# AberHu/TF-NAS

Measured on AMD Instinct MI355X. Metric: supernet search images/sec (w-step + alpha-step), higher is better.
Workload: dtype fp32

## Files before the change

### tf-nas_amd/csrc/capi.hip

```cpp
#include <string.h>
#include "tfnas_dev.h"
#include "kernels.h"
#include "cell_impl.h"

#include <stdlib.h>
#include <mutex>
#include <vector>

struct SideCtx {
    int device;
    hipStream_t main, side;
    hipEvent_t fork[4], join;
};
static std::mutex g_side_mu;
static std::vector<SideCtx*> g_side;

static SideCtx* side_for(hipStream_t s) {
    int dev = 0;
    if (hipGetDevice(&dev) != hipSuccess) return nullptr;
    std::lock_guard<std::mutex> lk(g_side_mu);
    for (SideCtx* c : g_side)
        if (c->main == s && c->device == dev) return c;
    SideCtx* c = new SideCtx();
    c->device = dev;
// ... 246 lines not shown
    if (bn) TRY(bn_fwd_fix(d0, bn, 1, stats2, s));
    TRY(launch_se_pool(d, b.D, stats2, pooled, s));
    TRY(launch_se_fc_fwd(d, pooled, hpre, gate, b.part, TFNAS_PART_FLOATS, s));
    TRY(launch_project_fwd(d, b.D, gate, stats2, b.Pr, stats3, b.part, s));
    if (sync) TRY(stats_sync(d, stats3, 2 * (size_t)d.G * d.oc, s));
    if (bn) TRY(bn_fwd_fix(d0, bn, 2, stats3, s));
    if (b.drop_scale && d.has_res) {
        TfnasCellDesc dn = dc;
        dn.has_res = 0;
        TRY(launch_mix_fwd(dn, b.Pr, stats3, b.wmix, b.x, b.out, s));
        return launch_rowscale(b.out, b.out, b.x, b.drop_scale, d.N, (uint64_t)d.Ho * d.Wo * d.oc, s);
    }
    TRY(launch_mix_fwd(d, b.Pr, stats3, b.wmix, b.x, b.out, s));
    return 0;
}

static hipStream_t fork_to(const CellSide* so, int k, hipStream_t main) {
    if (!so || !so->side[k] || so->side[k] == main) return main;
    if (hipEventRecord(so->fork[k], main) != hipSuccess || hipStreamWaitEvent(so->side[k], so->fork[k], 0) != hipSuccess)
        return main;
    return so->side[k];
}

static int bn_bwd_fix(const TfnasCellDesc& d, const TfnasBnAffine* bn, int site, double* red, hipStream_t s) {
    int nch;
    uint64_t cnt;
    bn_site(d, site, nch, cnt);
    TRY(launch_bn_bwd_fix(red, nch, cnt, bn->weight[site], bn->bias[site], bn->g_weight[site], bn->g_bias[site], s,
                          wgrad_accum(d)));
    if (bn->eval) return (int)hipMemsetAsync(red, 0, sizeof(double) * 2 * (size_t)nch, s);
    return 0;
}

static int expand_dx(const TfnasCellDesc& d, const float* dEh, const float* x, const float* cb1, float* part, const float* dout,
                     const float* wmix, float* dx, float* dxp, hipStream_t s, const float* add_src = nullptr,
                     const float* add_scale = nullptr, int nsl = -1) {
    const size_t room = TFNAS_PART_FLOATS - expand_gram_floats(d);
    float* gram = part + room;
    TRY(launch_expand_gram(d, cb1, part, room, gram, s));
    return launch_expand_dgrad(d, dEh, x, cb1, gram, dout, wmix, dx, dxp, s, add_src, add_scale, nsl);
}


int cell_bwd_impl(const TfnasCellDesc& d0, const TfnasCellWs& ws, const CellBwdBufs& b0, hipStream_t s, const CellSide* so,
                  int fwd_route) {
    const TfnasBnAffine* bn = b0.bn;
    TfnasCellDesc dc = d0;
    if (bn) dc.eps = -1.f;
    const TfnasCellDesc& d = dc;
    CellBwdBufs b = b0;
    const int taken = route_taken(d0, bn != nullptr);
    if ((fwd_route & TFNAS_ROUTE_TAKEN_VALID) && taken != fwd_route) return TFNAS_EINVAL;
    const float* dout_res = b0.dout;
    if (b0.drop_scale && d.has_res) {
        if (!b0.dout_s) return TFNAS_ENULL;
        TRY(launch_rowscale(b0.dout_s, b0.dout, nullptr, b0.drop_scale, d.N, (uint64_t)d.Ho * d.Wo * d.oc, s));
        b.dout = b0.dout_s;
    }
    const double* stats1 = b.stats + ws.off_stats1;
    const double* stats2 = b.stats + ws.off_stats2;
    const double* stats3 = b.stats + ws.off_stats3;
    const float* pooled = b.fsmall + ws.off_pooled;
    const float* gate = b.fsmall + ws.off_gate;
    const float* hpre = b.fsmall + ws.off_hpre;
    float* dgate = b.bsmall + ws.off_dgate;
    float* dpooled = b.bsmall + ws.off_dpooled;
    float* dhpre = b.bsmall + ws.off_dhpre;
    float* cb1 = b.bsmall + ws.off_cb1;
    double* red3 = b.red + ws.off_red3;
    double* red2 = b.red + ws.off_red2;
    double* red1 = b.red + ws.off_red1;
    float* part = b.part;
    float* part_w = b.part_w;
    float* part_w1 = b.part_w1 ? b.part_w1 : b.part_w;
    float* part_w2 = b.part_w2 ? b.part_w2 : b.part_w;

    if (d.need_wgrad) {
        for (int g = 0; g < d.G; ++g) {
            const TfnasGroup& gr = d.g[g];
            if (!gr.g_expand || !gr.g_dw || !gr.g_proj) return TFNAS_ENULL;
            if (gr.se > 0 && (!gr.g_se_r || !gr.gb_se_r || !gr.g_se_e || !gr.gb_se_e)) return TFNAS_ENULL;
        }
    }
    TRY(launch_mix_bwd_stats(d, b.dout, b.Pr, stats3, b.x, red3, part, s));
    TRY(stats_sync(d, red3, 2 * (size_t)d.G * d.oc, s));
    if (b.dwmix) TRY(launch_mix_dw(d, red3, b.red + ws.off_resdot, b.dwmix, s));
    if (bn) TRY(bn_bwd_fix(d0, bn, 2, red3, s));
    if (!b.dx && !d.need_wgrad) return 0;
    if (d.need_wgrad)
        TRY(launch_project_wgrad(d, b.dout, b.Pr, b.D, gate, stats2, stats3, red3, b.wmix, part_w, fork_to(so, 0, s)));
    const bool fused2 = bn2_fused_fits(d);
    const bool fold = fused2 && !(d.route & TFNAS_ROUTE_FOLD_OFF) && project_fold_ok(d, (size_t)ws.dEh) && (d.G == 1 || d.Ho * d.Wo <= 784);
    if (fold) {
        TRY(launch_project_dgrad(d, b.dout, b.Pr, stats3, red3, b.wmix, b.dZ, s, b.D, stats2, b.dEh));
        TRY(launch_bn2_gather(d, b.dEh, dgate, part, s));
    } else {
        TRY(launch_project_dgrad(d, b.dout, b.Pr, stats3, red3, b.wmix, b.dZ, s));
        if (fused2) TRY(launch_bn2_pool(d, b.dZ, b.D, stats2, dgate, part, s));
        else TRY(launch_se_bwd_reduce(d, b.dZ, b.D, stats2, dgate, s));
    }
    TRY(launch_se_fc_bwd(d, dgate, gate, hpre, dhpre, dpooled, b.dEh, (size_t)ws.dEh, s));
    if (fused2) TRY(launch_bn2_finish(d, part, gate, dpooled, red2, s));
    else TRY(launch_bn2_bwd(d, b.dZ, b.D, stats2, gate, dpooled, red2, part, s));
    TRY(stats_sync(d, red2, 2 * (size_t)d.M, s));
    if (bn) TRY(bn_bwd_fix(d0, bn, 1, red2, s));
    if (taken & TFNAS_ROUTE_TAKEN_FX) {
        int nsl = 0;
        TRY(launch_fx_bwd(d, b.x, b.E, stats1, stats2, red2, b.dZ, b.D, gate, dpooled, b.dEh, (size_t)ws.dEh, red1, cb1, part, &nsl, s));
        if (b.dx) TRY(expand_dx(d, nullptr, b.x, cb1, part, dout_res, b.wmix, b.dx, b.dEh, s, b.add_src, b.add_scale, nsl));
        return 0;
    }
    const DwPlan dw_bwd = dw_plan_bwd_data(d, b.E == nullptr, b.x != nullptr);
    const bool dw_fused = dw_bwd.fuse_wgrad;
    if (d.need_wgrad) {
        if (d.SE > 0 || !dw_fused) {
            hipStream_t sw = fork_to(so, 1, s);
            if (d.SE > 0) TRY(launch_se_wgrad(d, dgate, gate, dhpre, hpre, pooled, sw));
            if (!dw_fused) TRY(launch_dw_wgrad(d, b.dZ, gate, dpooled, b.D, stats2, red2, b.E, stats1, part_w1, sw));
        }
    }
    if (bn || stats_sync_on(d)) {
        TRY(launch_dw_bwd_data(dw_bwd, d, b.dZ, gate, dpooled, b.D, stats2, red2, b.E, b.x, stats1, b.dEh, red1, part, s));
        TRY(stats_sync(d, red1, 2 * (size_t)d.M, s));
        if (bn) TRY(bn_bwd_fix(d0, bn, 0, red1, s));
        TRY(launch_bn1_consts(d, stats1, red1, cb1, s));
    } else {
        TRY(launch_dw_bwd_data(dw_bwd, d, b.dZ, gate, dpooled, b.D, stats2, red2, b.E, b.x, stats1, b.dEh, red1, part, s, cb1));
    }
    if (d.need_wgrad) TRY(launch_expand_wgrad(d, b.dEh, b.E, cb1, b.x, part_w2, fork_to(so, 2, s)));
    if (b.dx && d.mode != TFNAS_MODE_STEM)
        TRY(expand_dx(d, b.dEh, b.x, cb1, part, dout_res, b.wmix, b.dx, b.dxp, s, b.add_src, b.add_scale));
    return 0;
}

extern "C" int tfnas_mixedop_fwd(const TfnasCellDesc* dp, const float* x, const float* wmix, float* E, float* D,
                                 float* Pr, float* fsmall, double* stats, float* part, float* out, void* stream) {
    if (!dp || !x || !D || !Pr || !fsmall || !stats || !part || !out) return TFNAS_ENULL;
    const TfnasCellDesc& d = *dp;
    if (d.mode == TFNAS_MODE_HEAD) return TFNAS_EINVAL;
    if (!E && !efree_supported(d)) return TFNAS_ENULL;
    TRY(check_modes(dp));
    TfnasCellWs ws;
    TRY(tfnas_cell_ws(dp, &ws));
    CellFwdBufs b = {x, wmix, E, D, Pr, fsmall, stats, part, out};
    return cell_fwd_impl(d, ws, b, S(stream));
}

static int cell_bwd_entry(const TfnasCellDesc& d, CellBwdBufs b, hipStream_t s, void* const* wgrad_stream, bool lazy) {
    TfnasCellWs ws;
    TRY(tfnas_cell_ws(&d, &ws));
    SideCtx* sc = (d.need_wgrad && route_side(d)) ? side_for(s) : nullptr;
    SideJoinGuard guard;
    guard.c = sc;
    guard.main = s;
    CellSide so = {};
    if (sc) {
        for (int i = 0; i < 3; ++i) {
            hipStream_t own = (wgrad_stream && wgrad_stream[i]) ? S(wgrad_stream[i]) : nullptr;
            so.side[i] = own ? own : sc->side;
            guard.extra[i] = own;
            so.fork[i] = sc->fork[i];
            if (own) {
                b.part_w1 = b.part + 2 * TFNAS_PART_ALLOC;
                b.part_w2 = b.part + 3 * TFNAS_PART_ALLOC;
            }
        }
    }
// ... 195 lines not shown
```

### tf-nas_amd/csrc/kernels.h

```cpp
#pragma once
#include <stdlib.h>
#include <hip/hip_runtime.h>
#include "tfnas_hip.h"

struct StatsSync {
    tfnas_stats_sync_fn fn;
    void* user;
    int world;
};
extern StatsSync g_stats_sync;
static inline StatsSync sync_of(const TfnasCellDesc& d) {
    if (d.sync_fn) return StatsSync{d.sync_fn, d.sync_user, d.sync_world > 0 ? d.sync_world : 1};
    return g_stats_sync;
}
static inline bool stats_sync_on(const TfnasCellDesc& d) { return sync_of(d).fn != nullptr; }
static inline int stats_sync(const TfnasCellDesc& d, double* table, size_t ndoubles, hipStream_t s) {
    const StatsSync y = sync_of(d);
    return y.fn ? y.fn(y.user, table, (uint64_t)ndoubles, (void*)s) : 0;
}
static inline uint64_t stats_world(const TfnasCellDesc& d) {
    const StatsSync y = sync_of(d);
    return (y.fn && y.world > 1) ? (uint64_t)y.world : 1;
}

// ... 35 lines not shown
                         const double* red3, const float* wmix, float* dZ, hipStream_t s, const float* D = nullptr,
                         const double* stats2 = nullptr, float* rec = nullptr);
constexpr int FOLD_SLOTS = 4, FOLD_Q = 5;
static inline bool project_fold_ok(const TfnasCellDesc& d, size_t scratch_floats) {
    const int HW = d.Ho * d.Wo;
    const size_t nrt = ((size_t)d.N * HW + 127) / 128;
    return HW >= 43 && nrt * FOLD_SLOTS * FOLD_Q * (size_t)d.M <= scratch_floats;
}
int launch_project_wgrad(const TfnasCellDesc& d, const float* dout, const float* Pr, const float* D,
                         const float* gate, const double* stats2, const double* stats3, const double* red3,
                         const float* wmix, float* part, hipStream_t s);
size_t expand_gram_floats(const TfnasCellDesc& d);
int launch_expand_gram(const TfnasCellDesc& d, const float* cb1, float* scratch, size_t scratch_floats, float* gram,
                       hipStream_t s);
int launch_expand_dgrad(const TfnasCellDesc& d, const float* dEh, const float* x, const float* cb1, const float* gram,
                        const float* dout, const float* wmix, float* dx, float* dxp, hipStream_t s,
                        const float* add_src = nullptr, const float* add_scale = nullptr, int nsl = -1);
int launch_expand_wgrad(const TfnasCellDesc& d, const float* dEh, const float* E, const float* cb1,
                        const float* x, float* part, hipStream_t s);

struct DwDirect {
    int chunks;
    int ncg;
    int nseg;
    int per;
    int steps;
    int nwg;
};
struct DwSlide {
    int TH, TW;
    int CC, CCP, cq_shift;
    int RB, L1;
    int chunks, gx;
};
struct DwGeom {
    int T0, T1;
    int CC;
    int cq_shift;
    int tilesH, tilesW, ntiles;
    int L0, L1;
};
enum DwFamily { DW_DIRECT, DW_RING, DW_TILE };
struct DwPlan {
    DwFamily fam;
    int rows;
    int chunks[2];
    DwDirect direct[2];
    DwSlide ring[2];
    DwGeom tile[2];
    int jw;
    bool pipe;
    int kq;
    bool fuse_wgrad;
};
int launch_dw_fwd(const TfnasCellDesc& d, const float* E, const float* x, const double* stats1, float* D,
                  double* stats2, float* part, hipStream_t s);
bool efree_supported(const TfnasCellDesc& d);
static inline bool efree_ic_ok(int ic) { return ic == 16 || ic == 24 || ic == 40; }
int launch_expand_stats_gram(const TfnasCellDesc& d, const float* x, double* stats1, float* part, hipStream_t s);
int launch_x_colsum(const float* x, int P, int ic, int rps, int nb, float* part, hipStream_t s);
bool fx_supported(const TfnasCellDesc& d);
int launch_fx_stats(const TfnasCellDesc& d, const float* x, double* stats1, float* part, hipStream_t s);
int launch_fx_fwd(const TfnasCellDesc& d, const float* x, const double* stats1, float* E, float* D, double* stats2,
                  float* part, hipStream_t s);
int launch_fx_bwd(const TfnasCellDesc& d, const float* x, const float* Eh, const double* stats1, const double* stats2,
                  const double* red2, const float* dZ, const float* D, const float* gate, const float* dpooled, float* scratch,
                  size_t scratch_floats, double* red1, float* cb1, float* part, int* nsl, hipStream_t s);
DwPlan dw_plan_bwd_data(const TfnasCellDesc& d, bool efree, bool has_x);
int launch_dw_bwd_data(const DwPlan& p, const TfnasCellDesc& d, const float* dZ, const float* gate, const float* dpooled,
                       const float* D, const double* stats2, const double* red2, const float* E, const float* x,
                       const double* stats1, float* dEh, double* red1, float* part, hipStream_t s, float* cb1 = nullptr);
int launch_reduce_bn1(const TfnasCellDesc& d, const float* part, int nb, const double* stats1, double* red1, float* cb1,
                      hipStream_t s);
int launch_dw_wgrad(const TfnasCellDesc& d, const float* dZ, const float* gate, const float* dpooled, const float* D,
                    const double* stats2,
                    const double* red2, const float* E, const double* stats1, float* part, hipStream_t s);

int launch_se_pool(const TfnasCellDesc& d, const float* D, const double* stats2, float* pooled, hipStream_t s);
int launch_se_fc_fwd(const TfnasCellDesc& d, const float* pooled, float* hpre, float* gate, float* scratch,
                     size_t scratch_floats, hipStream_t s);
int launch_mix_fwd(const TfnasCellDesc& d, const float* Pr, const double* stats3, const float* wmix,
                   const float* x, float* out, hipStream_t s);
int launch_mix_bwd_stats(const TfnasCellDesc& d, const float* dout, const float* Pr, const double* stats3,
                         const float* x, double* red3, float* part, hipStream_t s);
int launch_mix_dw(const TfnasCellDesc& d, const double* red3, const double* resdot, float* dwmix, hipStream_t s);
int launch_se_bwd_reduce(const TfnasCellDesc& d, const float* dZ, const float* D, const double* stats2,
                         float* dgate, hipStream_t s);
int launch_se_fc_bwd(const TfnasCellDesc& d, const float* dgate, const float* gate, const float* hpre, float* dhpre,
                     float* dpooled, float* scratch, size_t scratch_floats, hipStream_t s);
int launch_se_wgrad(const TfnasCellDesc& d, const float* dgate, const float* gate, const float* dhpre,
                    const float* hpre, const float* pooled, hipStream_t s);
bool bn2_fused_fits(const TfnasCellDesc& d);
int launch_bn2_pool(const TfnasCellDesc& d, const float* dZ, const float* D, const double* stats2, float* dgate,
                    float* pp, hipStream_t s);
int launch_bn2_gather(const TfnasCellDesc& d, const float* rec, float* dgate, float* pp, hipStream_t s);
int launch_bn2_finish(const TfnasCellDesc& d, const float* pp, const float* gate, const float* dpooled, double* red2,
                      hipStream_t s);
int launch_bn2_bwd(const TfnasCellDesc& d, const float* dZ, const float* D, const double* stats2, const float* gate,
                   const float* dpooled, double* red2, float* part, hipStream_t s);
int launch_head_pool(const TfnasCellDesc& d, const float* E, const double* stats1, float* pooled, hipStream_t s);
int launch_head_bwd(const TfnasCellDesc& d, const float* E, const double* stats1, const float* dpooled, float* dEh,
                    double* red1, float* part, hipStream_t s);
int launch_reduce_rows(const float* part, int nb, int ncols, size_t stride, double* out_d, float* out_f,
                       hipStream_t s, int accum = 0);
#define TFNAS_PART_ALLOC ((size_t)4 << 20)
#define TFNAS_TAIL_SLOTS ((size_t)1024)
#define TFNAS_PART_FLOATS (TFNAS_PART_ALLOC - TFNAS_TAIL_SLOTS)
int launch_bn1_consts(const TfnasCellDesc& d, const double* stats1, const double* red1, float* cb1,
                      hipStream_t s);

int launch_arch_fwd(int ncell, const float* const* la, const float* e, const float* lat, float T, float* w,
                    float* cell_lat, hipStream_t s);
int launch_arch_bwd(int ncell, const float* w, const float* lat, const float* dw, const float* dcl, float T,
                    float* const* dla, hipStream_t s);
int launch_arch_project(int n, float* const* p, const int32_t* len, hipStream_t s);
int launch_arch_sample(int ncell, const float* const* la, const uint8_t* mask, const float* e, float T, int mode,
                       int32_t* pos, hipStream_t s);
int launch_sink_fwd(int K, const float* betas, const float* const* res, const float* cell_lat, uint64_t count,
                    float* out, float* out_lat, float* bw, hipStream_t s);
int launch_scale_copy(float* dst, const float* src, const float* scale, uint64_t count, hipStream_t s);
int launch_sink_bwd(int K, const float* bw, const float* const* res, const float* cell_lat, const float* dout,
                    const float* dlat, uint64_t count, float* const* dres, float* dbetas, float* dcell_lat,
                    double* dots, hipStream_t s);

int launch_pack_ranges(const float* src, float* dst, int nranges, const uint64_t* off, const uint64_t* doff,
                       const uint64_t* len, hipStream_t s);
int launch_sgd_clip_step(float* w, float* g, float* m, int nranges, const uint64_t* off, const uint64_t* goff,
                         const uint64_t* len, float max_norm,
                         float lr, float momentum, float wd, float grad_scale, double* scratch, uint64_t scratch_doubles,
                         float* norm_out, hipStream_t s);
int launch_arch_adam_project(int n, float* const* p, const float* const* g, const int32_t* len, float* m, float* v,
                             float max_norm, float lr, float b1, float b2, float eps, float wd, int step, float grad_scale,
                             float* norm_out, hipStream_t s);

int launch_bn_fwd_fix(double* stats, int nch, uint64_t cnt, float eps, const float* gamma, const float* beta, float* rmean,
                      float* rvar, float momentum, int eval, hipStream_t s, uint64_t world = 1);
int launch_bn_bwd_fix(double* red, int nch, uint64_t cnt, const float* gamma, const float* beta, float* dgamma, float* dbeta,
                      hipStream_t s, int accum = 0);
int launch_rowscale(float* out, const float* y, const float* res, const float* scale, int N, uint64_t per_image,
                    hipStream_t s);
```

### tf-nas_amd/csrc/pointwise_kernels.hip

```cpp
#include "tfnas_dev.h"
#include "kernels.h"
#include "prof.h"

__device__ __forceinline__ f32x4 reduce_rows(f32x4 v, f32x4* buf, int pr, int col, int RP, int TQ, bool active) {
    __syncthreads();
    if (active) buf[pr * TQ + col] = v;
    __syncthreads();
    int s = 1;
    while (s * 2 < RP) s *= 2;
    for (; s > 0; s >>= 1) {
        if (active && pr < s && pr + s < RP) buf[pr * TQ + col] += buf[(pr + s) * TQ + col];
        __syncthreads();
    }
    return (active && pr == 0) ? buf[col] : zero4();
}

__device__ __forceinline__ bool chunk_locate(const TfnasCellDesc& d, int cy, int CH, bool se_only, int& g, int& c0) {
    for (g = 0; g < d.G; ++g) {
        if (se_only && d.g[g].se == 0) continue;
        const int t = (d.g[g].mcp + CH - 1) / CH;
        if (cy < t) {
            c0 = cy * CH;
            return true;
        }
// ... 9 lines not shown
}
#ifndef TFNAS_POOL_ROWS
#define TFNAS_POOL_ROWS 4
#endif
constexpr int PU = TFNAS_POOL_ROWS;
template <int ACT, int MODE>
__global__ __launch_bounds__(256) void k_se_pool(TfnasCellDesc d, const float* __restrict__ D,
                                                 const double* __restrict__ stats2, const float* __restrict__ dZ,
                                                 float* __restrict__ outp) {
    __shared__ f32x4 buf[256];
    int g, c0;
    if (!chunk_locate(d, blockIdx.y, 64, true, g, c0)) return;
    const int mc = d.g[g].mc, mcp = d.g[g].mcp, off = d.g[g].off;
    const int HW = d.Ho * d.Wo, M = d.M, n = blockIdx.x;
    const int nq = (min(64, mcp - c0) + 3) >> 2, cqs = nq <= 4 ? 2 : (nq <= 8 ? 3 : 4), CQN = 1 << cqs, RLN = 256 >> cqs;
    const int tid = threadIdx.x, cq = tid & (CQN - 1), rl = tid >> cqs;
    const int ch = c0 + 4 * cq;
    const bool active = ch < mcp;
    float2 c2[4];
#pragma unroll
    for (int j = 0; j < 4; ++j)
        c2[j] = (active && ch + j < mc) ? bn_consts(stats2 + 2 * (size_t)(off + ch + j), 1.0 / ((double)d.N * HW), d.eps)
                                        : make_float2(0.f, 0.f);
    f32x4 acc = zero4();
    if (active) {
        for (int hw = rl; hw < HW; hw += PU * RLN) {
            f32x4 v[PU], z[PU];
#pragma unroll
            for (int u = 0; u < PU; ++u) {
                const int h = hw + RLN * u;
                const size_t a = ((size_t)n * HW + (h < HW ? h : 0)) * M + off + ch;
                v[u] = ld4_nt(D + a);
                z[u] = (MODE == 1) ? ld4_nt(dZ + a) : zero4();
            }
#pragma unroll
            for (int u = 0; u < PU; ++u) {
                if (hw + RLN * u < HW) {
#pragma unroll
                    for (int j = 0; j < 4; ++j) v[u][j] = act_f<ACT>((v[u][j] - c2[j].x) * c2[j].y);
                    acc += (MODE == 1) ? v[u] * z[u] : v[u];
                }
            }
        }
    }
    acc = reduce_rows(acc, buf, rl, cq, RLN, CQN, active);
    if (active && rl == 0) {
        if (MODE == 0) acc *= splat4(1.f / (float)HW);
        st4(outp + (size_t)n * M + off + ch, acc);
    }
}

__global__ __launch_bounds__(256) void k_mix_fwd(TfnasCellDesc d, const float* __restrict__ Pr,
                                                 const double* __restrict__ stats3, const float* __restrict__ wmix,
                                                 const float* __restrict__ x, float* __restrict__ out) {
    extern __shared__ __attribute__((aligned(16))) float lds[];
    float2* tab = reinterpret_cast<float2*>(lds);
    const int oc = d.oc, G = d.G, OQ = oc >> 2;
    const int Po = d.N * d.Ho * d.Wo;
    float sumw = 0.f;
    for (int g = 0; g < G; ++g) sumw += wmix ? wmix[g] : 1.f;
    for (int i = threadIdx.x; i < G * oc; i += 256) {
        const float2 c = bn_consts(stats3 + 2 * (size_t)i, 1.0 / (double)Po, d.eps);
        tab[i] = make_float2(c.x, c.y * (wmix ? wmix[i / oc] : 1.f));
    }
    __syncthreads();
    const size_t total = (size_t)Po * OQ;
    for (size_t idx = (size_t)blockIdx.x * 256 + threadIdx.x; idx < total; idx += (size_t)gridDim.x * 256) {
        const size_t p = idx / OQ;
        const int o = (int)(idx % OQ) * 4;
        f32x4 v = zero4();
        for (int g = 0; g < G; ++g) {
            const f32x4 pr = ld4(Pr + ((size_t)g * Po + p) * oc + o);
#pragma unroll
            for (int j = 0; j < 4; ++j) {
                const float2 t = tab[g * oc + o + j];
                v[j] += (pr[j] - t.x) * t.y;
            }
        }
        if (d.has_res) v += splat4(sumw) * ld4(x + p * d.ic + o);
        st4(out + p * oc + o, v);
    }
}

__global__ __launch_bounds__(256) void k_mix_bwd_stats(TfnasCellDesc d, const float* __restrict__ dout,
                                                       const float* __restrict__ Pr,
                                                       const double* __restrict__ stats3,
                                                       const float* __restrict__ x, float* __restrict__ part,
                                                       int rows_per_block) {
    extern __shared__ __attribute__((aligned(16))) float lds[];
    const int oc = d.oc, TQ = oc >> 2, RP = 256 / TQ;
    const int Po = d.N * d.Ho * d.Wo;
    const int G = d.G, Gall = d.G;
    float2* tab = reinterpret_cast<float2*>(lds);
    f32x4* buf = reinterpret_cast<f32x4*>(lds + 2 * Gall * oc);
    for (int i = threadIdx.x; i < G * oc; i += 256) tab[i] = bn_consts(stats3 + 2 * (size_t)i, 1.0 / (double)Po, d.eps);
    __syncthreads();
    const int tid = threadIdx.x, oq = tid % TQ, pr = tid / TQ, o = 4 * oq;
    const bool active = pr < RP;
    const int p0 = blockIdx.x * rows_per_block, p1 = min(Po, p0 + rows_per_block);
    f32x4 s1 = zero4(), sx = zero4(), s2[TFNAS_MAX_GROUPS];
#pragma unroll
    for (int g = 0; g < TFNAS_MAX_GROUPS; ++g) s2[g] = zero4();
    if (active) {
        for (int p = p0 + pr; p < p1; p += RP) {
            const f32x4 dv = ld4(dout + (size_t)p * oc + o);
            s1 += dv;
            if (d.has_res) sx += dv * ld4(x + (size_t)p * d.ic + o);
#pragma unroll
            for (int g = 0; g < TFNAS_MAX_GROUPS; ++g) {
                if (g < G) {
                    const f32x4 pv = ld4(Pr + ((size_t)g * Po + p) * oc + o);
#pragma unroll
                    for (int j = 0; j < 4; ++j) {
                        const float2 t = tab[g * oc + o + j];
                        s2[g][j] += dv[j] * ((pv[j] - t.x) * t.y);
                    }
                }
            }
        }
    }
    float* prow = part + (size_t)blockIdx.x * (2 * Gall * oc + oc);
    s1 = reduce_rows(s1, buf, pr, oq, RP, TQ, active);
    sx = reduce_rows(sx, buf, pr, oq, RP, TQ, active);
    if (active && pr == 0) st4(prow + 2 * Gall * oc + o, sx);
#pragma unroll
    for (int g = 0; g < TFNAS_MAX_GROUPS; ++g) {
        if (g < G) {
            const f32x4 r = reduce_rows(s2[g], buf, pr, oq, RP, TQ, active);
            if (active && pr == 0) {
#pragma unroll
                for (int j = 0; j < 4; ++j) {
                    prow[2 * ((size_t)g * oc + o + j) + 0] = s1[j];
                    prow[2 * ((size_t)g * oc + o + j) + 1] = r[j];
                }
            }
        }
    }
}

__global__ __launch_bounds__(64) void k_mix_dw(TfnasCellDesc d, const double* __restrict__ red3, const double* __restrict__ resdot,
                                               float* __restrict__ dwmix) {
    const int g = blockIdx.x, lane = threadIdx.x;
    double s = 0.0;
    for (int o = lane; o < d.oc; o += 64) {
        s += red3[2 * ((size_t)g * d.oc + o) + 1];
        if (d.has_res) s += resdot[o];
    }
#pragma unroll
    for (int m = 32; m > 0; m >>= 1) s += __shfl_xor(s, m, 64);
    if (lane == 0) dwmix[g] = (float)s;
}

template <int ACT>
__global__ __launch_bounds__(256) void k_bn2_pool(TfnasCellDesc d, const float* __restrict__ dZ, const float* __restrict__ D,
                                                  const double* __restrict__ stats2, float* __restrict__ dgate,
                                                  float* __restrict__ pp, int CH) {
    __shared__ f32x4 buf[256];
    int g, c0;
    if (!chunk_locate(d, blockIdx.y, CH, false, g, c0)) return;
    const int mc = d.g[g].mc, mcp = d.g[g].mcp, off = d.g[g].off;
    const bool has_se = d.g[g].se > 0;
    const int HW = d.Ho * d.Wo, M = d.M, n = blockIdx.x;
    const int nq = (min(CH, mcp - c0) + 3) >> 2, cqs = nq <= 4 ? 2 : (nq <= 8 ? 3 : 4), CQN = 1 << cqs, RLN = 256 >> cqs;
    const int tid = threadIdx.x, cq = tid & (CQN - 1), rl = tid >> cqs;
    const int ch = c0 + 4 * cq;
    const bool active = ch < mcp;
    float2 c2[4];
#pragma unroll
    for (int j = 0; j < 4; ++j)
        c2[j] = (active && ch + j < mc) ? bn_consts(stats2 + 2 * (size_t)(off + ch + j), 1.0 / ((double)d.N * HW), d.eps)
                                        : make_float2(0.f, 0.f);
    f32x4 g0 = zero4(), a1 = zero4(), b1 = zero4(), a2 = zero4(), b2 = zero4();
    if (active) {
        for (int hw = rl; hw < HW; hw += PU * RLN) {
            f32x4 v[PU], z[PU];
#pragma unroll
            for (int u = 0; u < PU; ++u) {
                const int h = hw + RLN * u;
                const size_t a = ((size_t)n * HW + (h < HW ? h : 0)) * M + off + ch;
                v[u] = ld4_nt(D + a);
                z[u] = ld4_nt(dZ + a);
            }
#pragma unroll
            for (int u = 0; u < PU; ++u) {
                if (hw + RLN * u < HW) {
#pragma unroll
                    for (int j = 0; j < 4; ++j) {
                        const float dh = (v[u][j] - c2[j].x) * c2[j].y;
                        const float ad = act_d<ACT>(dh), zd = z[u][j] * ad;
                        a1[j] += zd;
                        b1[j] += zd * dh;
                        if (has_se) {
                            g0[j] += z[u][j] * act_f<ACT>(dh);
                            a2[j] += ad;
                            b2[j] += ad * dh;
                        }
                    }
                }
            }
        }
    }
    const size_t NM = (size_t)d.N * M, o = (size_t)n * M + off + ch;
    a1 = reduce_rows(a1, buf, rl, cq, RLN, CQN, active);
    if (active && rl == 0) st4(pp + o, a1);
    b1 = reduce_rows(b1, buf, rl, cq, RLN, CQN, active);
    if (active && rl == 0) st4(pp + NM + o, b1);
    if (has_se) {
        a2 = reduce_rows(a2, buf, rl, cq, RLN, CQN, active);
        if (active && rl == 0) st4(pp + 2 * NM + o, a2);
        b2 = reduce_rows(b2, buf, rl, cq, RLN, CQN, active);
        if (active && rl == 0) st4(pp + 3 * NM + o, b2);
        g0 = reduce_rows(g0, buf, rl, cq, RLN, CQN, active);
        if (active && rl == 0) st4(dgate + o, g0);
    }
}

__global__ __launch_bounds__(256) void k_bn2_gather(TfnasCellDesc d, const float* __restrict__ rec, float* __restrict__ dgate,
                                                    float* __restrict__ pp) {
// ... 389 lines not shown
    __syncthreads();
    if (tid < CL / 2) {
        const int ch = blockIdx.x * (CL / 2) + tid;
        if (ch < d.M) {
            const double inv = 1.0 / ((double)d.N * d.H * d.W);
            const float2 m = bn_consts(stats1 + 2 * (size_t)ch, inv, d.eps);
            f32x4 t;
            t.x = m.x;
            t.y = m.y;
            t.z = (float)(tot[2 * tid] * inv);
            t.w = (float)(tot[2 * tid + 1] * inv);
            bool is_pad = true;
            for (int g = 0; g < d.G; ++g)
                if (ch >= d.g[g].off && ch < d.g[g].off + d.g[g].mc) is_pad = false;
            if (is_pad) t = zero4();
            reinterpret_cast<f32x4*>(cb1)[ch] = t;
        }
    }
}

int launch_reduce_bn1(const TfnasCellDesc& d, const float* part, int nb, const double* stats1, double* red1, float* cb1,
                      hipStream_t s) {
    ProfScope _prof(TK_REDUCE_ROWS, s);
    hipLaunchKernelGGL(k_reduce_bn1, dim3(cdiv(2 * d.M, 16)), dim3(256), 0, s, d, part, nb, stats1, red1, cb1);
    return (int)hipGetLastError();
}

int launch_reduce_rows(const float* part, int nb, int ncols, size_t stride, double* out_d, float* out_f,
                       hipStream_t s, int accum) {
    ProfScope _prof(TK_REDUCE_ROWS, s);
    const bool al4 = (ncols & 3) == 0 && (stride & 3) == 0 && ((uintptr_t)part & 15) == 0;
    const size_t in_stride = 0, out_stride = 0;
    if (al4 && nb <= 128 && ncols >= 1024)
        hipLaunchKernelGGL(k_reduce_rows_wide, dim3(cdiv(ncols, 128), 1), dim3(256), 0, s, part, nb, ncols, stride, out_d,
                           out_f, in_stride, out_stride, accum);
    else if (al4 && nb > 64)
        hipLaunchKernelGGL(k_reduce_rows_q<4>, dim3(cdiv(ncols, 16), 1), dim3(256), 0, s, part, nb, ncols, stride, out_d, out_f,
                           in_stride, out_stride, accum);
    else if (ncols <= 2048 && nb > 256)
        hipLaunchKernelGGL(k_reduce_rows<4>, dim3(cdiv(ncols, 4), 1), dim3(256), 0, s, part, nb, ncols, stride, out_d, out_f,
                           in_stride, out_stride, accum);
    else
        hipLaunchKernelGGL(k_reduce_rows<8>, dim3(cdiv(ncols, 8), 1), dim3(256), 0, s, part, nb, ncols, stride, out_d, out_f,
                           in_stride, out_stride, accum);
    return (int)hipGetLastError();
}

int launch_se_pool(const TfnasCellDesc& d, const float* D, const double* stats2, float* pooled, hipStream_t s) {
    ProfScope _prof(TK_SE_POOL, s);
    const int chunks = chunk_count(d, 64, true);
    if (!chunks) return 0;
    dim3 grid(d.N, chunks);
    ACT_DISPATCH(d.act, {
        hipLaunchKernelGGL((k_se_pool<ACT, 0>), grid, dim3(256), 0, s, d, D, stats2, (const float*)nullptr, pooled);
    })
    return (int)hipGetLastError();
}

int launch_se_bwd_reduce(const TfnasCellDesc& d, const float* dZ, const float* D, const double* stats2,
                         float* dgate, hipStream_t s) {
    ProfScope _prof(TK_SE_BWD_REDUCE, s);
    const int chunks = chunk_count(d, 64, true);
    if (!chunks) return 0;
    dim3 grid(d.N, chunks);
    ACT_DISPATCH(d.act, {
        hipLaunchKernelGGL((k_se_pool<ACT, 1>), grid, dim3(256), 0, s, d, D, stats2, dZ, dgate);
    })
    return (int)hipGetLastError();
}

int launch_mix_fwd(const TfnasCellDesc& d, const float* Pr, const double* stats3, const float* wmix,
                   const float* x, float* out, hipStream_t s) {
    ProfScope _prof(TK_MIX_FWD, s);
    const size_t total = (size_t)d.N * d.Ho * d.Wo * (d.oc / 4);
    size_t blocks = cdiv64(total, 256 * 4);
    if (blocks > 4096) blocks = 4096;
    if (blocks < 1) blocks = 1;
    const size_t shm = (size_t)2 * d.G * d.oc * sizeof(float);
    hipLaunchKernelGGL(k_mix_fwd, dim3((unsigned)blocks), dim3(256), shm, s, d, Pr, stats3, wmix, x, out);
    return (int)hipGetLastError();
}

int launch_mix_bwd_stats(const TfnasCellDesc& d, const float* dout, const float* Pr, const double* stats3,
                         const float* x, double* red3, float* part, hipStream_t s) {
    ProfScope _prof(TK_MIX_BWD_STATS, s);
    const int Po = d.N * d.Ho * d.Wo;
    const int ncols = 2 * d.G * d.oc + d.oc;
    size_t nblk = 1024;
    if (nblk > TFNAS_PART_FLOATS / (size_t)ncols) nblk = TFNAS_PART_FLOATS / (size_t)ncols;
    int rpb = cdiv(Po, (int)nblk);
    const int RP = 256 / (d.oc / 4);
    if (rpb < 8 * RP) rpb = 8 * RP;
    const size_t shm = (size_t)(2 * d.G * d.oc + 4 * 256) * sizeof(float);
    const int gx = cdiv(Po, rpb);
    hipLaunchKernelGGL(k_mix_bwd_stats, dim3(gx), dim3(256), shm, s, d, dout, Pr, stats3, x, part, rpb);
    _prof.stop();
    return launch_reduce_rows(part, gx, ncols, (size_t)ncols, red3, nullptr, s);
}

int launch_mix_dw(const TfnasCellDesc& d, const double* red3, const double* resdot, float* dwmix, hipStream_t s) {
    ProfScope _prof(TK_SMALL, s);
    hipLaunchKernelGGL(k_mix_dw, dim3(d.G), dim3(64), 0, s, d, red3, resdot, dwmix);
    return (int)hipGetLastError();
}

int launch_bn2_bwd(const TfnasCellDesc& d, const float* dZ, const float* D, const double* stats2, const float* gate,
                   const float* dpooled, double* red2, float* part, hipStream_t s) {
    ProfScope _prof(TK_BN2_BWD, s);
    const int Po = d.N * d.Ho * d.Wo;
    const int chunks = chunk_count(d, 64, false);
    int want = cdiv(4096, chunks);
    if (want > 1024) want = 1024;
    const size_t cap = TFNAS_PART_FLOATS / (2 * (size_t)d.M);
    if ((size_t)want > cap) want = (int)cap;
    int rpb = cdiv(Po, want < 1 ? 1 : want);
    if (rpb < 64) rpb = 64;
    dim3 grid(cdiv(Po, rpb), chunks);
    ACT_DISPATCH(d.act, {
        hipLaunchKernelGGL((k_bn2_bwd<ACT>), grid, dim3(256), 0, s, d, dZ, D, stats2, gate, dpooled, part, rpb);
    })
    _prof.stop();
    return launch_reduce_rows(part, grid.x, 2 * d.M, 2 * (size_t)d.M, red2, nullptr, s);
}

bool bn2_fused_fits(const TfnasCellDesc& d) { return 4 * (size_t)d.N * d.M <= TFNAS_PART_FLOATS; }

int launch_bn2_pool(const TfnasCellDesc& d, const float* dZ, const float* D, const double* stats2, float* dgate,
                    float* pp, hipStream_t s) {
    ProfScope _prof(TK_SE_BWD_REDUCE, s);
    const int CH = (d.N * chunk_count(d, 64, false) < 1024 && d.Ho * d.Wo >= 196) ? 32 : 64;
    dim3 grid(d.N, chunk_count(d, CH, false));
    ACT_DISPATCH(d.act, { hipLaunchKernelGGL((k_bn2_pool<ACT>), grid, dim3(256), 0, s, d, dZ, D, stats2, dgate, pp, CH); })
    return (int)hipGetLastError();
}

int launch_bn2_gather(const TfnasCellDesc& d, const float* rec, float* dgate, float* pp, hipStream_t s) {
    ProfScope _prof(TK_SE_BWD_REDUCE, s);
    hipLaunchKernelGGL(k_bn2_gather, dim3(d.N, chunk_count(d, 64, false)), dim3(256), 0, s, d, rec, dgate, pp);
    return (int)hipGetLastError();
}

int launch_bn2_finish(const TfnasCellDesc& d, const float* pp, const float* gate, const float* dpooled, double* red2,
                      hipStream_t s) {
    ProfScope _prof(TK_BN2_BWD, s);
    hipLaunchKernelGGL(k_bn2_finish, dim3(chunk_count(d, 64, false)), dim3(256), 0, s, d, pp, gate, dpooled, red2);
    return (int)hipGetLastError();
}

int launch_head_pool(const TfnasCellDesc& d, const float* E, const double* stats1, float* pooled, hipStream_t s) {
    ProfScope _prof(TK_SMALL, s);
    dim3 grid(d.N, cdiv(d.g[0].mcp, 64));
    ACT_DISPATCH(d.act, { hipLaunchKernelGGL((k_head_pool<ACT>), grid, dim3(256), 0, s, d, E, stats1, pooled); })
    return (int)hipGetLastError();
}

int launch_head_bwd(const TfnasCellDesc& d, const float* E, const double* stats1, const float* dpooled, float* dEh,
                    double* red1, float* part, hipStream_t s) {
    ProfScope _prof(TK_SMALL, s);
    if ((size_t)d.N * 2 * d.M > TFNAS_PART_FLOATS) return TFNAS_ERANGE;
    dim3 grid(d.N, cdiv(d.g[0].mcp, 64));
    ACT_DISPATCH(d.act, { hipLaunchKernelGGL((k_head_bwd<ACT>), grid, dim3(256), 0, s, d, E, stats1, dpooled, dEh, part); })
    _prof.stop();
    return launch_reduce_rows(part, d.N, 2 * d.M, 2 * (size_t)d.M, red1, nullptr, s);
}

int launch_bn1_consts(const TfnasCellDesc& d, const double* stats1, const double* red1, float* cb1,
                      hipStream_t s) {
    ProfScope _prof(TK_SMALL, s);
    hipLaunchKernelGGL(k_bn1_consts, dim3(cdiv(d.M, 256)), dim3(256), 0, s, d, stats1, red1, cb1);
    return (int)hipGetLastError();
}
```

Before: 3870.

## Specialize mix backward-stats kernel by group count and compact its partial-sum layout

Templates the mix backward-stats kernel on the group count and on whether the residual dot product is needed, skipping the x read when dwmix is not requested. Each thread now issues several row loads before accumulating, to keep more memory requests in flight. Partials are stored once per column (s1 no longer duplicated per group) and reduced in LDS. A dedicated double-precision reduce kernel then scatters the sums into red3 and resdot. The cost is more template instances and more LDS per block; the pointer passed as resdot must match the workspace offset the caller reads.

```diff
diff --git a/tf-nas_amd/csrc/capi.hip b/tf-nas_amd/csrc/capi.hip
--- a/tf-nas_amd/csrc/capi.hip
+++ b/tf-nas_amd/csrc/capi.hip
@@ -352,7 +352,7 @@
             if (gr.se > 0 && (!gr.g_se_r || !gr.gb_se_r || !gr.g_se_e || !gr.gb_se_e)) return TFNAS_ENULL;
         }
     }
-    TRY(launch_mix_bwd_stats(d, b.dout, b.Pr, stats3, b.x, red3, part, s));
+    TRY(launch_mix_bwd_stats(d, b.dout, b.Pr, stats3, b.x, red3, part, b.dwmix != nullptr, s));
     TRY(stats_sync(d, red3, 2 * (size_t)d.G * d.oc, s));
     if (b.dwmix) TRY(launch_mix_dw(d, red3, b.red + ws.off_resdot, b.dwmix, s));
     if (bn) TRY(bn_bwd_fix(d0, bn, 2, red3, s));
diff --git a/tf-nas_amd/csrc/kernels.h b/tf-nas_amd/csrc/kernels.h
--- a/tf-nas_amd/csrc/kernels.h
+++ b/tf-nas_amd/csrc/kernels.h
@@ -141,7 +141,7 @@
 int launch_mix_fwd(const TfnasCellDesc& d, const float* Pr, const double* stats3, const float* wmix,
                    const float* x, float* out, hipStream_t s);
 int launch_mix_bwd_stats(const TfnasCellDesc& d, const float* dout, const float* Pr, const double* stats3,
-                         const float* x, double* red3, float* part, hipStream_t s);
+                         const float* x, double* red3, float* part, bool want_resdot, hipStream_t s);
 int launch_mix_dw(const TfnasCellDesc& d, const double* red3, const double* resdot, float* dwmix, hipStream_t s);
 int launch_se_bwd_reduce(const TfnasCellDesc& d, const float* dZ, const float* D, const double* stats2,
                          float* dgate, hipStream_t s);
diff --git a/tf-nas_amd/csrc/pointwise_kernels.hip b/tf-nas_amd/csrc/pointwise_kernels.hip
--- a/tf-nas_amd/csrc/pointwise_kernels.hip
+++ b/tf-nas_amd/csrc/pointwise_kernels.hip
@@ -115,58 +115,114 @@
     }
 }
 
+constexpr int mix_rows_in_flight(int G) { return G == 1 ? 8 : (G <= 3 ? 4 : 2); }
+
+template <int G, bool WX>
 __global__ __launch_bounds__(256) void k_mix_bwd_stats(TfnasCellDesc d, const float* __restrict__ dout,
                                                        const float* __restrict__ Pr,
                                                        const double* __restrict__ stats3,
                                                        const float* __restrict__ x, float* __restrict__ part,
                                                        int rows_per_block) {
     extern __shared__ __attribute__((aligned(16))) float lds[];
+    constexpr int U = mix_rows_in_flight(G), NA = 1 + (WX ? 1 : 0) + G;
     const int oc = d.oc, TQ = oc >> 2, RP = 256 / TQ;
     const int Po = d.N * d.Ho * d.Wo;
-    const int G = d.G, Gall = d.G;
     float2* tab = reinterpret_cast<float2*>(lds);
-    f32x4* buf = reinterpret_cast<f32x4*>(lds + 2 * Gall * oc);
+    float* stage = lds + 2 * G * oc;
     for (int i = threadIdx.x; i < G * oc; i += 256) tab[i] = bn_consts(stats3 + 2 * (size_t)i, 1.0 / (double)Po, d.eps);
     __syncthreads();
     const int tid = threadIdx.x, oq = tid % TQ, pr = tid / TQ, o = 4 * oq;
     const bool active = pr < RP;
     const int p0 = blockIdx.x * rows_per_block, p1 = min(Po, p0 + rows_per_block);
-    f32x4 s1 = zero4(), sx = zero4(), s2[TFNAS_MAX_GROUPS];
-#pragma unroll
-    for (int g = 0; g < TFNAS_MAX_GROUPS; ++g) s2[g] = zero4();
+    f32x4 s1 = zero4(), sx = zero4(), s2[G];
+#pragma unroll
+    for (int g = 0; g < G; ++g) s2[g] = zero4();
     if (active) {
-        for (int p = p0 + pr; p < p1; p += RP) {
-            const f32x4 dv = ld4(dout + (size_t)p * oc + o);
-            s1 += dv;
-            if (d.has_res) sx += dv * ld4(x + (size_t)p * d.ic + o);
-#pragma unroll
-            for (int g = 0; g < TFNAS_MAX_GROUPS; ++g) {
-                if (g < G) {
-                    const f32x4 pv = ld4(Pr + ((size_t)g * Po + p) * oc + o);
+        for (int pb = p0 + pr; pb < p1; pb += U * RP) {
+            f32x4 dv[U], xv[U], pv[U][G];
+#pragma unroll
+            for (int u = 0; u < U; ++u) {
+                const int p = pb + u * RP < p1 ? pb + u * RP : pb;
+                dv[u] = ld4(dout + (size_t)p * oc + o);
+                if (WX) xv[u] = ld4(x + (size_t)p * d.ic + o);
+#pragma unroll
+                for (int g = 0; g < G; ++g) pv[u][g] = ld4(Pr + ((size_t)g * Po + p) * oc + o);
+            }
+#pragma unroll
+            for (int u = 0; u < U; ++u) {
+                if (pb + u * RP >= p1) dv[u] = zero4();
+                s1 += dv[u];
+                if (WX) {
+#pragma unroll
+                    for (int j = 0; j < 4; ++j) sx[j] = __builtin_fmaf(dv[u][j], xv[u][j], sx[j]);
+                }
+#pragma unroll
+                for (int g = 0; g < G; ++g) {
 #pragma unroll
                     for (int j = 0; j < 4; ++j) {
                         const float2 t = tab[g * oc + o + j];
-                        s2[g][j] += dv[j] * ((pv[j] - t.x) * t.y);
+                        const float ph = (pv[u][g][j] - t.x) * t.y;
+                        s2[g][j] = __builtin_fmaf(dv[u][j], ph, s2[g][j]);
                     }
                 }
             }
         }
-    }
-    float* prow = part + (size_t)blockIdx.x * (2 * Gall * oc + oc);
-    s1 = reduce_rows(s1, buf, pr, oq, RP, TQ, active);
-    sx = reduce_rows(sx, buf, pr, oq, RP, TQ, active);
-    if (active && pr == 0) st4(prow + 2 * Gall * oc + o, sx);
-#pragma unroll
-    for (int g = 0; g < TFNAS_MAX_GROUPS; ++g) {
-        if (g < G) {
-            const f32x4 r = reduce_rows(s2[g], buf, pr, oq, RP, TQ, active);
-            if (active && pr == 0) {
-#pragma unroll
-                for (int j = 0; j < 4; ++j) {
-                    prow[2 * ((size_t)g * oc + o + j) + 0] = s1[j];
-                    prow[2 * ((size_t)g * oc + o + j) + 1] = r[j];
-                }
-            }
+        f32x4* st = reinterpret_cast<f32x4*>(stage) + pr * TQ + oq;
+        const int plane = RP * TQ;
+        st[0] = s1;
+        if (WX) st[plane] = sx;
+#pragma unroll
+        for (int g = 0; g < G; ++g) st[(1 + (WX ? 1 : 0) + g) * plane] = s2[g];
+    }
+    __syncthreads();
+    float* prow = part + (size_t)blockIdx.x * (NA * oc);
+    int top = 1;
+    while (top * 2 < RP) top *= 2;
+    for (int c = tid; c < NA * oc; c += 256) {
+        const int a = c / oc, oo = c - a * oc;
+        float* col = stage + (size_t)a * RP * oc + oo;
+        for (int s = top; s > 0; s >>= 1)
+            for (int r = 0; r < s; ++r)
+                if (r + s < RP) col[r * oc] += col[(r + s) * oc];
+        prow[c] = col[0];
+    }
+}
+
+__global__ __launch_bounds__(256) void k_mix_reduce(TfnasCellDesc d, const float* __restrict__ part, int nb, int wx,
+                                                    double* __restrict__ red3, double* __restrict__ resdot) {
+    constexpr int QN = 4, RL = 256 / QN;
+    __shared__ double buf[RL][4 * QN + 2];
+    const int oc = d.oc, G = d.G, nfc = (1 + wx + G) * oc;
+    const int tid = threadIdx.x;
+    const int cq = tid % QN, rl = tid / QN;
+    const int c = (blockIdx.x * QN + cq) * 4;
+    double s[4] = {0.0, 0.0, 0.0, 0.0};
+    if (c < nfc) {
+        for (int b = rl; b < nb; b += 8 * RL) {
+            f32x4 v[8];
+#pragma unroll
+            for (int u = 0; u < 8; ++u) v[u] = (b + RL * u < nb) ? ld4(part + (size_t)(b + RL * u) * nfc + c) : zero4();
+#pragma unroll
+            for (int j = 0; j < 4; ++j)
+                s[j] += (((double)v[0][j] + (double)v[1][j]) + ((double)v[2][j] + (double)v[3][j])) +
+                        (((double)v[4][j] + (double)v[5][j]) + ((double)v[6][j] + (double)v[7][j]));
+        }
+    }
+#pragma unroll
+    for (int j = 0; j < 4; ++j) buf[rl][4 * cq + j] = s[j];
+    __syncthreads();
+    const int cc = blockIdx.x * 4 * QN + tid;
+    if (tid < 4 * QN && cc < nfc) {
+        double t = 0.0;
+#pragma unroll
+        for (int r = 0; r < RL; ++r) t += buf[r][tid];
+        const int a = cc / oc, oo = cc - a * oc;
+        if (a == 0) {
+            for (int g = 0; g < G; ++g) red3[2 * ((size_t)g * oc + oo)] = t;
+        } else if (wx && a == 1) {
+            resdot[oo] = t;
+        } else {
+            red3[2 * ((size_t)(a - 1 - wx) * oc + oo) + 1] = t;
         }
     }
 }
@@ -722,20 +778,38 @@
 }
 
 int launch_mix_bwd_stats(const TfnasCellDesc& d, const float* dout, const float* Pr, const double* stats3,
-                         const float* x, double* red3, float* part, hipStream_t s) {
+                         const float* x, double* red3, float* part, bool want_resdot, hipStream_t s) {
     ProfScope _prof(TK_MIX_BWD_STATS, s);
-    const int Po = d.N * d.Ho * d.Wo;
-    const int ncols = 2 * d.G * d.oc + d.oc;
+    const int Po = d.N * d.Ho * d.Wo, G = d.G, oc = d.oc;
+    if (G < 1 || G > TFNAS_MAX_GROUPS || (oc & 3) || oc > 1024) return TFNAS_ERANGE;
+    const int wx = (want_resdot && d.has_res) ? 1 : 0;
+    const int nfc = (1 + wx + G) * oc;
+    const int widest = 2 * G * oc + oc;
     size_t nblk = 1024;
-    if (nblk > TFNAS_PART_FLOATS / (size_t)ncols) nblk = TFNAS_PART_FLOATS / (size_t)ncols;
+    if (nblk > TFNAS_PART_FLOATS / (size_t)widest) nblk = TFNAS_PART_FLOATS / (size_t)widest;
     int rpb = cdiv(Po, (int)nblk);
-    const int RP = 256 / (d.oc / 4);
+    const int RP = 256 / (oc / 4);
     if (rpb < 8 * RP) rpb = 8 * RP;
-    const size_t shm = (size_t)(2 * d.G * d.oc + 4 * 256) * sizeof(float);
+    const size_t shm = ((size_t)2 * G * oc + (size_t)(1 + wx + G) * RP * oc) * sizeof(float);
     const int gx = cdiv(Po, rpb);
-    hipLaunchKernelGGL(k_mix_bwd_stats, dim3(gx), dim3(256), shm, s, d, dout, Pr, stats3, x, part, rpb);
+#define MIX_STATS_CASE(GG)                                                                                                   \
+    case GG:                                                                                                                 \
+        if (wx) hipLaunchKernelGGL((k_mix_bwd_stats<GG, true>), dim3(gx), dim3(256), shm, s, d, dout, Pr, stats3, x, part,  \
+                                   rpb);                                                                                     \
+        else hipLaunchKernelGGL((k_mix_bwd_stats<GG, false>), dim3(gx), dim3(256), shm, s, d, dout, Pr, stats3, x, part,    \
+                                rpb);                                                                                        \
+        break;
+    switch (G) {
+        MIX_STATS_CASE(1) MIX_STATS_CASE(2) MIX_STATS_CASE(3) MIX_STATS_CASE(4)
+        MIX_STATS_CASE(5) MIX_STATS_CASE(6) MIX_STATS_CASE(7) MIX_STATS_CASE(8)
+    }
+#undef MIX_STATS_CASE
     _prof.stop();
-    return launch_reduce_rows(part, gx, ncols, (size_t)ncols, red3, nullptr, s);
+    const int rc = (int)hipGetLastError();
+    if (rc) return rc;
+    ProfScope _prof2(TK_REDUCE_ROWS, s);
+    hipLaunchKernelGGL(k_mix_reduce, dim3(cdiv(nfc, 16)), dim3(256), 0, s, d, part, gx, wx, red3, red3 + 2 * (size_t)G * oc);
+    return (int)hipGetLastError();
 }
 
 int launch_mix_dw(const TfnasCellDesc& d, const double* red3, const double* resdot, float* dwmix, hipStream_t s) {
```

Result: no change. 3899 (median of 6 runs) (+0.7%).
